# jchibane/Box2Mask

Measured on AMD Instinct MI355X. Metric: ScanNet scenes/sec (fwd+bwd, ~150k voxels @2cm), higher is better.
Workload: dtype f32; 1 GPU; ScanNet 2cm voxels, batch_size=8 per GPU, sparse-conv fwd/bwd + losses + Adam (BASELINE configs[1]); global_batch=8, ranks_seen=1, voxels_per_gpu_batch=1202778, parallelism=dp1, distinct_batches=4, setup_steps=2, prefetch=next batch: coordinate + kernel maps on a second stream during the step, steps_executed=51, full=False

## Files before the change

box2mask_amd/_lib.py:

```python
from __future__ import annotations

import ctypes as C
import os

import torch

_HERE = os.path.dirname(os.path.abspath(__file__))
LIB_PATH = os.environ.get('B2M_LIB_PATH', os.path.join(_HERE, 'libb2m_hip.so'))

P = C.c_void_p
I32 = C.c_int32
I64 = C.c_int64
F32 = C.c_float
F64 = C.c_double

PROTOTYPES = {
    'b2m_coords_build': [P, I64, P, P, I64, P, P],
    'b2m_morton_keys': [P, I64, P, P],
    'b2m_hilbert_keys': [P, I64, I32, P, P],
    'b2m_coords_stride': [P, I64, I32, P, P, P, P, P, I64, P, C.POINTER(I64), P],
    'b2m_kernel_map': [P, I64, I32, I32, P, P, I64, P, I32, I32, I32, P, I64, P],
    'b2m_occupancy': [P, I64, I32, I32, I32, I32, P, I64, P],
    'b2m_kernel_map_rulebook': [P, I64, I32, I32, P, P, I64, P, I32, I32, I32, P, P, P, P],
    'b2m_stride_tables': [P, P, I64, I64, P, I64, P, I64, P],
# ... 21 lines not shown
    'b2m_weight_pack_run': [P, I32, I64, P],
    'b2m_weight_pack_h_run': [P, I32, I64, P],
    'b2m_conv_wgrad': [P, I64, I32, I64, P, I64, I32, P, P, P, I64, I32, P, I64, I64, P, P],
    'b2m_conv_wgrad_tr': [P, I64, I32, I64, P, I64, I32, P, P, P, I64, I32, P, I64, I64, P, P],
    'b2m_bn_stats': [P, I64, I64, I32, P, P, P],
    'b2m_bn_tilestats': [P, I64, I32, P, P, P],
    'b2m_bn_tilestats_finalize': [P, I64, I64, I32, P, P, P, P, F32, F32, P, P, P, P, P, P, P],
    'b2m_bn_finalize': [P, F64, P, I32, P, P, F32, F32, P, P, P, P, P, P, P],
    'b2m_bn_apply': [P, I64, I64, I32, P, P, P, I64, I32, P, I64, P],
    'b2m_bn_bwd_reduce': [P, I64, P, I64, P, I64, I64, I32, P, P, I32, P, P, P, P, P, P, P],
    'b2m_bn_stats_finalize': [P, I64, I64, I32, P, P, P, P, F32, F32, P, P, P, P, P, P, P],
    'b2m_bn_bwd_apply': [P, I64, P, I64, P, I64, I64, I32, P, P, P, P, F64, P, I32, P, P, P, I64, P, I64, P],
    'b2m_bn_apply2': [P, I64, P, I64, I64, I32, P, P, P, P, I32, P, I64, P],
    'b2m_bn_bwd_reduce2': [P, I64, P, I64, P, I64, P, I64, I64, I32, P, P, P, P, I32, P, P, P],
    'b2m_bn_bwd_apply2': [P, I64, P, I64, P, I64, P, I64, I64, I32, P, P, P, P, P, P, P, F64, P, I32, P, I64, P, I64, P, P, P, P, P, P],
    'b2m_bn_small_fwd': [P, I64, I64, I32, P, P, F32, F32, P, P, P, P, P, P, P, I64, I32, P, I64, P],
    'b2m_bn_small_fwd_stats': [P, I64, I64, I32, P, P],
    'b2m_bn_small_fwd_apply': [P, P, I64, I64, I32, P, P, F32, F32, P, P, P, P, P, P, P, I64, I32, P, I64, P],
    'b2m_bn_small_bwd_phase': [I32, P, I64, P, I64, P, I64, I64, I32, P, P, P, I32, P, P, P, P, P, I64, P, I64, P, P, P],
    'b2m_bn_small_bwd': [P, I64, P, I64, P, I64, I64, I32, P, P, P, I32, P, P, P, P, P, I64, P, I64, P],
    'b2m_relu_fwd': [P, I64, P, P],
    'b2m_relu_bwd': [P, P, I64, P, P],
    'b2m_add': [P, P, I64, P, P],
    'b2m_segment_pool_fwd': [P, I64, I64, I32, P, I64, I32, P, P, P, P, P],
    'b2m_segment_mean_sorted': [P, I64, I64, I32, P, P, I64, P, P, P],
    'b2m_segment_pool_bwd': [P, I64, I32, P, I64, I32, P, P, P, I64, P],
    'b2m_nmc': [P, I32, F32, I32, P, P, P, P, P, P],
    'b2m_nmc_batch': [P, P, I32, I32, F32, P, P, P, P, P, P],
    'b2m_mask_project': [P, I32, P, I32, P, P, I64, F32, P, I64, P],
    'b2m_mask_nms': [P, I32, I64, F32, P, P, P, P],
    'b2m_label_hist': [P, I64, P, I32, P, I64, I32, P, P],
    'b2m_mask_gather': [P, I64, P, I32, P, I64, P, P],
    'b2m_mask_project_batch': [P, I32, I64, I64, F32, P],
    'b2m_mask_nms_batch': [P, I32, I32, F32, P],
    'b2m_label_hist_batch': [P, I32, I64, I32, P],
    'b2m_mask_gather_batch': [P, I32, I64, I64, P],
    'b2m_mask_gather_batch_t': [P, I32, I64, I64, I64, P, P],
    'b2m_mask_nms_sweep': [P, I32, I64, P, I32, P, P, P],
    'b2m_mask_nms_sweep_batch': [P, I32, I32, P, I32, P, I64, P],
    'b2m_mask_hist_index': [P, I64, I32, I64, P, P, I64, I32, P, P, P],
    'b2m_mask_hist_index_batch': [P, I32, I64, I64, P],
    'b2m_mask_hist': [P, I64, I32, P, I64, I32, P, P],
    'b2m_mask_pack': [P, I32, I64, P, I64, P],
    'b2m_set_ious': [P, P, I64, P, P],
    'b2m_mask_hulls': [P, I64, I32, P, I64, P, P, P, I32, P, P, P, P, P, P, P],
    'b2m_obb_corners': [P, P, P, I32, P, P],
    'b2m_hull_box_iou': [P, P, P, P, I32, P, P, I32, P, P],
    'b2m_aabb_iou': [P, P, I32, P, P, P, I32, P, P],
    'b2m_dbscan': [P, I64, I32, F64, I32, P, P, P, P],
    'b2m_paint_proposals': [P, I64, I32, P, I64, I32, F64, I32, P, P, P, P, P],
    'b2m_joint_hist': [P, P, I64, I32, I32, P, P],
    'b2m_vox_shift': [P, I64, P, P, P],
    'b2m_unique_insert_async': [P, I64, P, I64, P, P, P, P],
    'b2m_vox_keys': [P, I64, P, F64, P, P, P],
    'b2m_sort_u64': [P, I64, P],
    'b2m_unique_rank': [P, I64, P, P, I64, P, I64, P, P],
    'b2m_vox_decode': [P, I64, I32, P, P],
    'b2m_vox_nearest': [P, I64, P, F64, P, P, I64, I64, P, P, P],
    'b2m_vox_gather': [P, I64, P, P, P, P, P, P],
    'b2m_seg_centroid': [P, P, I64, I64, F64, P, P, P, P, P],
    'b2m_box_membership': [P, I64, P, P, P, I32, P, P, P, P],
    'b2m_seg_box_vote': [P, I64, P, P, I64, I64, P, P, P, P, I32, P, P, P, P, P],
    'b2m_obb_membership': [P, I64, P, P, P, I32, P, P, P],
    'b2m_seg_rank': [P, I64, P, P, I64, P, P],
    'b2m_seg_mode': [P, P, I64, I64, I32, P, P, P],
    'b2m_aug_stats': [P, I64, P, P, P],
    'b2m_aug_affine': [P, P, I64, P, P, P, P, I32, P],
    'b2m_aug_axpy': [P, P, F64, I64, P],
    'b2m_aug_blur': [P, P, I32, I32, I32, P],
    'b2m_aug_displace': [P, I64, P, I32, I32, I32, P, P, P, F64, P],
    'b2m_aug_vertex_normals': [P, I64, P, I64, P, P, P, P],
    'b2m_aug_colour': [P, I64, P, I32, F64, P, P, P],
    'b2m_inst_boxes': [P, P, P, I64, I64, P, P, P, P, P, P, P, P, P, P],
    'b2m_nn_build': [P, I64, P, P],
    'b2m_nn_query': [P, I64, P, P, I64, P, P, P],
    'b2m_ap_rows': [P, I32, I32, P],
    'b2m_ap_match': [P, I32, I64, P, P, P, I32, P, I64, P, P, P, I64, P, P, P, I32, P],
    'b2m_ap_curve': [P, I64, P, P, I32, P, I64, I64, P, P, P, P],
}
PLAIN = {'b2m_last_error': (C.c_char_p, []), 'b2m_version': (C.c_int, []), 'b2m_device_ok': (C.c_int, []),
         'b2m_reload_env': (C.c_int, []),
         'b2m_weight_pack_size': (C.c_int64, [I32, I32, I32]),
         'b2m_conv_wgrad_workspace': (C.c_int64, [I32, I32, I32]),
         'b2m_weight_pack_h_size': (C.c_int64, [I32, I32, I32, I32]),
         'b2m_unique_insert': (C.c_int64, [P, I64, P, I64, P, P, P, P]),
         'b2m_weight_pack_plan_size': (C.c_int32, []),
         'b2m_weight_pack_h_plan_size': (C.c_int32, []),
         'b2m_weight_pack_h_plan': (C.c_int64, [I32, P, P, P, P, P, P, P, P, P, P, P]),
         'b2m_rulebook_cnt_size': (C.c_int64, [I32, I64]),
         'b2m_radix_argsort_scratch': (C.c_int64, [I64]),
         'b2m_dbscan_workspace': (C.c_int64, [I64]),
         'b2m_nn_workspace': (C.c_int64, [I64]),
         'b2m_xchg_size': (C.c_int64, []), 'b2m_xchg_max_doubles': (C.c_int32, []), 'b2m_xchg_max_ranks': (C.c_int32, []),
         'b2m_xchg_alloc': (C.c_int, [C.POINTER(C.c_void_p), P]), 'b2m_xchg_open': (C.c_int, [P, C.POINTER(C.c_void_p)]),
         'b2m_xchg_close': (C.c_int, [P]), 'b2m_xchg_free': (C.c_int, [P]),
         'b2m_xchg_is_finegrained': (C.c_int32, [P]),
         'b2m_weight_pack_plan': (C.c_int64, [I32, P, P, P, P, P, P, P, P, P, P, P])}

_lib = None


class B2MError(RuntimeError):
    pass


def load():
    global _lib
    if _lib is not None:
        return _lib
    if not os.path.exists(LIB_PATH):
        raise ImportError(
            'box2mask_amd: the HIP extension %s is missing. Build it with '
            '`python -m box2mask_amd.build` (hipcc --offload-arch=gfx950); there is no CPU fallback.' % LIB_PATH)
    lib = C.CDLL(LIB_PATH)
    for name, args in PROTOTYPES.items():
        fn = getattr(lib, name)
        fn.argtypes = args
        fn.restype = C.c_int
    for name, (res, args) in PLAIN.items():
        fn = getattr(lib, name)
        fn.argtypes = args
        fn.restype = res
    _lib = lib
    return lib


def ptr(t):
    if t is None:
        return None
    return t.data_ptr()


_raw_stream = getattr(torch._C, '_cuda_getCurrentRawStream', None)
_raw_device = getattr(torch._C, '_cuda_getDevice', None)


def stream():
    if _raw_stream is not None and _raw_device is not None:
        return _raw_stream(_raw_device())
    return torch.cuda.current_stream().cuda_stream


_hook = None


def set_hook(fn):
    global _hook
    _hook = fn


def call(name, *args, meta=None):
    lib = _lib if _lib is not None else load()
    done = _hook(name, args, meta) if _hook is not None else None
    rc = getattr(lib, name)(*args, stream())
    if done is not None:
        done()
    if rc != 0:
        raise B2MError('%s failed (%d): %s' % (name, rc, lib.b2m_last_error().decode()))


def call_ret(name, *args):
    lib = load()
    done = _hook(name, args, None) if _hook is not None else None
    rc = getattr(lib, name)(*args, stream())
    if done is not None:
        done()
# ... 18 lines not shown
```

box2mask_amd/csrc/conv.hip:

```cpp
#include "b2m_common.h"
#include <stdlib.h>
#include <type_traits>

struct ConvArgs {
    const float* x1; int64_t ldx1; int c1;
    const float* x2; int64_t ldx2; int c2;
    const float* wp; int K;
    const float* bias;
    const int32_t* rb_in; const uint8_t* rb_out; const int32_t* rb_cnt;
    int64_t n_out, ntiles;
    float* y; int64_t ldy; int cout; int accumulate; int nstrips; int vec_store;
    int nslice;
    int chain;
    int fast32;
    const float* zeros;
    int ncs;
    int wg_combine;
    int64_t nwg;
    int64_t xcd_per;
    const int32_t* xcd_start;
    int64_t wg_per_tile;
    const int32_t* tile_order;
    double* stats;
    const float* ep_scale; const float* ep_shift; const float* ep_res; int64_t ld_res; int ep_relu;
// ... 509 lines not shown
        bool more = true;
        while (more) {
#pragma unroll
            for (int u = 0; u < 3; ++u) {
                if (k0 < 0) { more = false; break; }
                const int n = count_of(k0);
                const int G = (n + 15) >> 4;
                const int k2c = valid(k2, valid(k1, k0)), k3c = valid(k3, k2c);
                load_ops(k2c, idx, av[(u + 2) % 3], w[(u + 2) % 3]);
                load_idx(k3c, idx);
                f32x4 acc[NG][TW];
#pragma unroll
                for (int g = 0; g < NG; ++g) {
                    if (g < G) {
#pragma unroll
                        for (int t = 0; t < TW; ++t) {
                            f32x4 c = {0.f, 0.f, 0.f, 0.f};
                            c = __builtin_amdgcn_mfma_f32_16x16x4f32(av[u][g][0], w[u][t], c, 0, 0, 0);
                            acc[g][t] = __builtin_amdgcn_mfma_f32_16x16x4f32(av[u][g][1], w[u][2 + t], c, 0, 0, 0);
                        }
                    }
                }
#pragma unroll
                for (int g = 0; g < NG; ++g) {
                    if (g < G) {
                        int ad[4];
                        float old[4][TW];
#pragma unroll
                        for (int r = 0; r < 4; ++r) {
                            ad[r] = (16 * g + 4 * q + r < n) ? (int)((out[u][g] >> (8 * r)) & 255) : B2M_TILE;
#pragma unroll
                            for (int t = 0; t < TW; ++t) old[r][t] = Cs[cs_index<TW>(ad[r], 16 * t + i)];
                        }
#pragma unroll
                        for (int r = 0; r < 4; ++r)
#pragma unroll
                            for (int t = 0; t < TW; ++t) Cs[cs_index<TW>(ad[r], 16 * t + i)] = old[r][t] + acc[g][t][r];
                    }
                }
                load_out(k3c, out[u]);
                k0 = k1; k1 = k2; k2 = k3;
                k3 = k2 < 0 ? -1 : next_active(k2);
            }
        }
        __builtin_amdgcn_fence(__ATOMIC_SEQ_CST, "wavefront");
    }
    if (a.stats && lane < a.cout) {
        const int64_t rem = a.n_out - row0;
        const int rows = rem < B2M_TILE ? (int)rem : B2M_TILE;
        double s1[4] = {0., 0., 0., 0.}, s2[4] = {0., 0., 0., 0.};
        int r = 0;
        for (; r + 3 < rows; r += 4) {
#pragma unroll
            for (int u = 0; u < 4; ++u) {
                const double v = (double)Cs[cs_index<TW>(r + u, lane)];
                s1[u] += v; s2[u] = fma(v, v, s2[u]);
            }
        }
        for (; r < rows; ++r) {
            const double v = (double)Cs[cs_index<TW>(r, lane)];
            s1[0] += v; s2[0] = fma(v, v, s2[0]);
        }
        double* o = a.stats + tile * 2 * a.cout + lane;
        o[0] = (s1[0] + s1[1]) + (s1[2] + s1[3]); o[a.cout] = (s2[0] + s2[1]) + (s2[2] + s2[3]);
    }
    for (int e = lane; e < B2M_TILE * (SW / 4); e += 64) {
        const int row = e / (SW / 4), c4 = (e % (SW / 4)) * 4;
        const int64_t grow = row0 + row;
        if (grow >= a.n_out) continue;
        f32x4 v = *(const f32x4*)&Cs[cs_index<TW>(row, c4)];
        float* dst = a.y + grow * a.ldy + c4;
        if (a.vec_store && c4 + 3 < a.cout) {
            if constexpr (EP) v = conv_epilogue(a, v, grow, c4);
            *(f32x4*)dst = v;
        } else {
#pragma unroll
            for (int u = 0; u < 4; ++u) if (c4 + u < a.cout) dst[u] = v[u];
        }
    }
}

#include "conv_fwd_flow.h"
#include "conv_1x1.h"

static inline int conv_kc(int cin) { return cin >= 16 ? 16 : 8; }
static inline int conv_tw(int cout, int K) { return (cout % 48 == 0 && K > 1 && b2m_env_int("B2M_CONV_TW3", 1)) ? 3 : 2; }

extern "C" int64_t b2m_weight_pack_size(int32_t K, int32_t cin, int32_t cout) {
    const int KC = conv_kc(cin);
    const int TW = conv_tw(cout, K);
    const int64_t nchunk = (cin + KC - 1) / KC, nstrip = (cout + 16 * TW - 1) / (16 * TW);
    return (int64_t)K * nstrip * nchunk * (64 * TW * (KC / 4));
}

__global__ void weight_pack_kernel(const float* __restrict__ w, int64_t ldw, int K, int rows, int cols, int transpose,
                                   int mirror, int sb, int CI, int CO, int KC, int TW, float* __restrict__ wp) {
    const int KS = KC / 4, LW = 64 * TW * KS, SW = 16 * TW;
    const int nchunk = (CI + KC - 1) / KC, nstrip = (CO + SW - 1) / SW;
    const int64_t total = (int64_t)K * nstrip * nchunk * LW;
    for (int64_t e = (int64_t)blockIdx.x * blockDim.x + threadIdx.x; e < total; e += (int64_t)gridDim.x * blockDim.x) {
        int lane, f;
        pack_unpos((int)(e % LW), TW * KS, lane, f);
        const int64_t blk = e / LW;
        const int chunk = (int)(blk % nchunk); const int64_t b2 = blk / nchunk;
        const int strip = (int)(b2 % nstrip); const int k = (int)(b2 / nstrip);
        const int s = f / TW, t = f % TW, q = lane >> 4, i = lane & 15;
        const int ci = chunk * KC + KS * q + s, co = strip * SW + 16 * t + i;
        float v = 0.f;
        if (ci < CI && co < CO) {
            if (!transpose) v = w[((int64_t)k * rows + ci) * ldw + co];
            else v = w[((int64_t)(mirror ? K - 1 - k : k) * rows + sb + co) * ldw + ci];
        }
        wp[e] = v;
    }
}
extern "C" int b2m_weight_pack(const float* w, int64_t ldw, int32_t K, int32_t cin, int32_t cout, int32_t transpose,
                               int32_t mirror, int32_t slice_begin, int32_t slice_count, float* wp, void* stream) {
    hipStream_t st = (hipStream_t)stream;
    B2M_CHECK_ARG(w && wp && K >= 1 && cin > 0 && cout > 0 && ldw >= cout, "bad arguments");
    int CI, CO;
    if (!transpose) { CI = cin; CO = cout; }
    else {
        B2M_CHECK_ARG(slice_begin >= 0 && slice_count > 0 && slice_begin + slice_count <= cin, "bad channel slice");
        CI = cout; CO = slice_count;
    }
    const int64_t total = b2m_weight_pack_size(K, CI, CO);
    int64_t grid = (total + 255) / 256;
    if (grid > 65536) grid = 65536;
    weight_pack_kernel<<<(unsigned)grid, 256, 0, st>>>(w, ldw, K, cin, cout, transpose, mirror, slice_begin, CI, CO,
                                                       conv_kc(CI), conv_tw(CO, K), wp);
    B2M_LAUNCH_CHECK();
    return B2M_OK;
}

struct PackDesc {
    const float* w; float* wp;
    int64_t ldw, first_block, total;
    int32_t K, rows, cols, transpose, mirror, sb, CI, CO, KC, TW;
};
extern "C" int32_t b2m_weight_pack_plan_size(void) { return (int32_t)sizeof(PackDesc); }
extern "C" int64_t b2m_weight_pack_plan(int32_t n, const int64_t* w, const int64_t* wp, const int64_t* ldw,
                                        const int32_t* K, const int32_t* cin, const int32_t* cout,
                                        const int32_t* transpose, const int32_t* mirror, const int32_t* slice_begin,
                                        const int32_t* slice_count, void* plan_host) {
    B2M_CHECK_ARG(n >= 0 && (n == 0 || (w && wp && ldw && K && cin && cout && transpose && mirror && slice_begin &&
                                        slice_count && plan_host)), "bad arguments");
    PackDesc* d = (PackDesc*)plan_host;
    int64_t blocks = 0;
    for (int i = 0; i < n; ++i) {
        B2M_CHECK_ARG(w[i] && wp[i] && K[i] >= 1 && cin[i] > 0 && cout[i] > 0 && ldw[i] >= cout[i], "bad layer");
        PackDesc e;
        e.w = (const float*)(uintptr_t)w[i]; e.wp = (float*)(uintptr_t)wp[i]; e.ldw = ldw[i];
        e.K = K[i]; e.rows = cin[i]; e.cols = cout[i]; e.transpose = transpose[i]; e.mirror = mirror[i]; e.sb = slice_begin[i];
        if (!transpose[i]) { e.CI = cin[i]; e.CO = cout[i]; }
        else {
            B2M_CHECK_ARG(slice_begin[i] >= 0 && slice_count[i] > 0 && slice_begin[i] + slice_count[i] <= cin[i], "bad channel slice");
            e.CI = cout[i]; e.CO = slice_count[i];
        }
        e.KC = conv_kc(e.CI); e.TW = conv_tw(e.CO, e.K);
        e.total = b2m_weight_pack_size(e.K, e.CI, e.CO);
        e.first_block = blocks;
        blocks += e.total / (64 * e.TW * (e.KC / 4));
        d[i] = e;
    }
    return blocks;
}
// ... 99 lines not shown
    return rows < (1 << 24) && ld < (1 << 22) && rows * ld * esz < (1ll << 32);
}
static inline bool addr32(int64_t rows, int64_t ld1, int64_t ld2, int esz) { return addr32(rows, ld1, esz) && addr32(rows, ld2, esz); }
static inline ConvArgs conv_args(const float* x1, int64_t ldx1, int c1, const float* x2, int64_t ldx2, int c2, const float* wp, int K,
                                 const int32_t* rb_in, const uint8_t* rb_out, const int32_t* rb_cnt, int64_t n_out, float* y, int64_t ldy,
                                 int cout, int TW) {
    ConvArgs a{};
    a.x1 = x1; a.ldx1 = ldx1; a.c1 = c1; a.x2 = x2; a.ldx2 = ldx2; a.c2 = c2;
    a.wp = wp; a.K = K;
    a.rb_in = rb_in; a.rb_out = rb_out; a.rb_cnt = rb_cnt;
    a.n_out = n_out; a.ntiles = cdiv64(n_out, B2M_TILE);
    a.y = y; a.ldy = ldy; a.cout = cout;
    a.nstrips = (cout + 16 * TW - 1) / (16 * TW);
    return a;
}
static inline unsigned conv_xcd_plan(ConvArgs& a, int64_t items_per_tile, int wpb, bool balanced) {
    const int64_t xcd_tiles = b2m_env_int("B2M_XCD", 1) ? (1 << 30) : 0;
    const XcdOrder o = xcd_order(a.nwg, xcd_tiles * items_per_tile / wpb);
    a.xcd_per = o.chunk;
    if (!(balanced && a.ntiles >= B2M_BALANCE_MIN_TILES && xcd_tiles > 0 && b2m_env_int("B2M_XCD_BALANCE", 1))) return o.grid;
    a.xcd_start = a.rb_cnt + (int64_t)a.K * a.ntiles;
    a.tile_order = b2m_env_int("B2M_XCD_ORDER", 1) ? a.xcd_start + 16 + a.ntiles : nullptr;
    a.wg_per_tile = items_per_tile / wpb;
    return (unsigned)(8 * B2M_XCD_CAP(a.ntiles) * a.wg_per_tile);
}

struct ConvEpilogue { const float* scale; const float* shift; const float* res; int64_t ld_res; int relu; };
static int conv_fwd_impl(const float* x1, int64_t ldx1, int32_t c1, const float* x2, int64_t ldx2, int32_t c2,
                         int64_t n_in, const float* wp, int32_t K, const float* bias, const int32_t* rb_in,
                         const uint8_t* rb_out, const int32_t* rb_cnt, int64_t n_out, float* y, int64_t ldy,
                         int32_t cout, int32_t accumulate, double* tile_stats, int32_t* wrote_stats, void* stream,
                         const ConvEpilogue* ep = nullptr, int32_t* fused = nullptr) {
    hipStream_t st = (hipStream_t)stream;
    if (wrote_stats) *wrote_stats = 0;
    if (fused) *fused = 0;
    B2M_CHECK_ARG(c1 > 0 && c2 >= 0 && cout > 0 && K >= 1 && K <= 128 && n_in >= 0 && n_out >= 0, "bad sizes (K<=128)");
    B2M_CHECK_ARG(ldy >= cout && ldx1 >= c1 && (c2 == 0 || ldx2 >= c2), "leading dimension too small");
    const int cin = c1 + c2;
    const int KC = conv_kc(cin);
    const int KS = KC / 4;
    B2M_CHECK_ARG(c2 == 0 || c1 % KC == 0, "with two sources c1 must be a multiple of 16");
    if (n_out == 0) return B2M_OK;
    B2M_CHECK_ARG(n_in >= 1, "n_in (rows of x1/x2) must be >= 1 where there are output rows");
    B2M_CHECK_ARG(x1 && wp && y, "bad pointers");
    B2M_CHECK_ARG((rb_in == nullptr) == (rb_out == nullptr) && (rb_in == nullptr) == (rb_cnt == nullptr),
                  "rulebook pointers must be all set or all NULL");
    B2M_CHECK_ARG(rb_in != nullptr || K == 1, "identity rulebook needs K == 1");
    B2M_CHECK_ARG(c2 == 0 || x2 != nullptr, "x2 is NULL");
    B2M_CHECK_ARG(((uintptr_t)wp % 16) == 0, "packed weights must be 16-byte aligned");
    const bool fast = c1 % KC == 0 && c2 % KC == 0 && ldx1 % KS == 0 && (c2 == 0 || ldx2 % KS == 0) &&
                      ((uintptr_t)x1 % (4 * KS)) == 0 && ((uintptr_t)x2 % (4 * KS)) == 0;
    const int TW = conv_tw(cout, K);
    ConvArgs a = conv_args(x1, ldx1, c1, x2, ldx2, c2, wp, K, rb_in, rb_out, rb_cnt, n_out, y, ldy, cout, TW);
    a.bias = bias; a.accumulate = accumulate;
    a.vec_store = (ldy % 4 == 0 && ((uintptr_t)y % 16) == 0) ? 1 : 0;
    const bool ep_ok = ep && ep->scale && ep->shift && a.vec_store && cout % 4 == 0 && !accumulate && !bias &&
                       ((uintptr_t)ep->scale % 16) == 0 && ((uintptr_t)ep->shift % 16) == 0 &&
                       (!ep->res || (ep->ld_res % 4 == 0 && ep->ld_res >= cout && ((uintptr_t)ep->res % 16) == 0));
    auto use_epilogue = [&]() {
        a.ep_scale = ep->scale; a.ep_shift = ep->shift; a.ep_res = ep->res; a.ld_res = ep->ld_res; a.ep_relu = ep->relu;
        if (fused) *fused = 1;
    };
    const int64_t items0 = a.ntiles * a.nstrips;
    int nslice = 1;
    const int64_t target = b2m_env_int("B2M_DETERMINISTIC", 0) ? 0 : b2m_env_int("B2M_CONV_TARGET", cin <= 32 ? 4096 : 6144);
    if (items0 < target && K > 1) {
        nslice = (int)cdiv64(target, items0);
        if (nslice > 16) nslice = 16;
        if (nslice > K) nslice = K;
        if (K >= 4 && nslice > 1) {
            nslice = (nslice + 3) / 4 * 4;
            if (nslice > K) nslice = K / 4 * 4;
            if (nslice > 16) nslice = 16;
            const int cap = b2m_env_int("B2M_CONV_MAXSLICE", a.ntiles >= 8 ? 4 : 16);
            if (nslice > cap) nslice = cap;
        }
    }
    int ncs = 1;
    const int nchunk_h = (cin + KC - 1) / KC;
    while (nslice > 1 && ncs < 4 && items0 * nslice * ncs < b2m_env_int("B2M_CONV_CHUNK_ITEMS", 2048) && nchunk_h / (ncs * 2) >= 2 &&
           b2m_env_int("B2M_CONV_CHUNKSPLIT", 1)) ncs *= 2;
    nslice *= ncs;
    a.fast32 = (addr32(n_in, ldx1, ldx2, 4) && b2m_env_int("B2M_CONV_FAST32", 1)) ? 1 : 0;
    bool split2 = false;
    if (nslice == 1 && K >= 8 && rb_in != nullptr && fast && KC == 16 && a.fast32 && (cin / 16) % 2 == 0 && cin >= 32 &&
        b2m_env_int("B2M_CONV_PIPE", 2) && b2m_env_int("B2M_CONV_HANDLOADS", 1) && !b2m_env_int("B2M_PIPE_DBG", 0) &&
        !b2m_env_int("B2M_DETERMINISTIC", 0) && items0 >= target && items0 < b2m_env_int("B2M_CONV_SPLIT2", 0)) {
        nslice = 2;
        split2 = true;
    }
    a.ncs = ncs;
    a.nslice = nslice;
    a.wg_combine = ((nslice > 1 && nslice % 4 == 0 && b2m_env_int("B2M_CONV_WGCOMBINE", 1)) || split2) ? 1 : 0;
    static const float* zeros_addr = nullptr;
    if (!zeros_addr) B2M_HIP(hipGetSymbolAddress((void**)&zeros_addr, HIP_SYMBOL(g_zeros)));
    a.zeros = zeros_addr;
    if (nslice > 1 && !accumulate && !(a.wg_combine && (nslice == 4 || split2)))
        B2M_HIP(hipMemset2DAsync(y, (size_t)ldy * sizeof(float), 0, (size_t)cout * sizeof(float), (size_t)n_out, st));
    const int64_t items = items0 * nslice;
    a.nwg = cdiv64(items, 4);
    const unsigned grid = conv_xcd_plan(a, (int64_t)a.nstrips * nslice, 4, false);
    const bool ident = rb_in == nullptr;
    if (ident && fast && KC == 16 && a.fast32 && n_in >= n_out && b2m_env_int("B2M_CONV_1X1", 1)) {
        int spw = a.nstrips % 3 == 0 ? 3 : a.nstrips % 2 == 0 ? 2 : 1;
        if (a.ntiles * (a.nstrips / spw) < 2048) spw = 1;
        const int64_t g1 = a.ntiles * (a.nstrips / spw);
        B2M_CHECK_ARG(g1 < (1ll << 31), "too many workgroups");
        if (ep_ok) use_epilogue();
        if (spw == 3) conv_1x1_kernel<3><<<(unsigned)g1, 64, 0, st>>>(a);
        else if (spw == 2) conv_1x1_kernel<2><<<(unsigned)g1, 64, 0, st>>>(a);
        else conv_1x1_kernel<1><<<(unsigned)g1, 64, 0, st>>>(a);
        B2M_LAUNCH_CHECK();
        return B2M_OK;
    }
    {
        const int nc = cin / 16;
        const int depth = b2m_env_int("B2M_CONV_PIPE", 2) ? 2 : 0;
        const bool split_ok = nslice == 1 || (a.wg_combine && b2m_env_int("B2M_CONV_FLOW_SPLIT", 1));
        if (depth >= 2 && !ident && fast && KC == 16 && split_ok && a.fast32 && nc % ncs == 0 && (nc / ncs) % depth == 0 &&
            nc / ncs >= depth) {
            const int wpb = nslice == 1 ? 1 : split2 ? 2 : 4;
            B2M_CHECK_ARG(items0 < (1ll << 31), "too many (tile, strip) items");
            a.chain = (wpb == 1 && b2m_env_int("B2M_CONV_CHAIN", 1)) ? 1 : 0;
            if (tile_stats && (nslice == 1 || ((nslice == 4 || split2) && !accumulate))) {
                a.stats = tile_stats;
                if (wrote_stats) *wrote_stats = 1;
            }
            if (ep_ok && (nslice == 1 || nslice == 4 || split2)) use_epilogue();
            a.nwg = cdiv64(items, wpb);
            const unsigned fgrid = conv_xcd_plan(a, (int64_t)a.nstrips * nslice, wpb, (a.nstrips * nslice) % wpb == 0);
            const int dbg = b2m_env_int("B2M_PIPE_DBG", 0);
            const int hl = b2m_env_int("B2M_CONV_HANDLOADS", 1);
            if (hl && depth == 2 && dbg == 32 && wpb == 1 && TW == 3) {
                conv_fwd_flow_kernel<2, 3, 32, 1, 1><<<fgrid, 64, 0, st>>>(a);
                B2M_LAUNCH_CHECK();
                return B2M_OK;
            }
            if (hl && depth == 2 && dbg == 8 && wpb == 1 && TW == 3) {
                conv_fwd_flow_kernel<2, 3, 8, 1, 1><<<fgrid, 64, 0, st>>>(a);
                B2M_LAUNCH_CHECK();
                return B2M_OK;
            }
            if (hl && depth == 2 && !dbg) {
                if (wpb == 2) {
                    if (TW == 3) conv_fwd_flow_kernel<2, 3, 0, 2, 1><<<fgrid, 128, 0, st>>>(a);
                    else conv_fwd_flow_kernel<2, 2, 0, 2, 1><<<fgrid, 128, 0, st>>>(a);
                } else if (wpb == 4) {
                    if (TW == 3) conv_fwd_flow_kernel<2, 3, 0, 4, 1><<<fgrid, 256, 0, st>>>(a);
                    else conv_fwd_flow_kernel<2, 2, 0, 4, 1><<<fgrid, 256, 0, st>>>(a);
                } else {
                    if (TW == 3) conv_fwd_flow_kernel<2, 3, 0, 1, 1><<<fgrid, 64, 0, st>>>(a);
                    else conv_fwd_flow_kernel<2, 2, 0, 1, 1><<<fgrid, 64, 0, st>>>(a);
                }
                B2M_LAUNCH_CHECK();
                return B2M_OK;
            }
            if (wpb == 4) {
                if (TW == 3) conv_fwd_flow_kernel<2, 3, 0, 4><<<fgrid, 256, 0, st>>>(a);
                else conv_fwd_flow_kernel<2, 2, 0, 4><<<fgrid, 256, 0, st>>>(a);
            } else if (dbg && TW == 3) {
                switch (dbg) {
                    case 1: conv_fwd_flow_kernel<2, 3, 1><<<fgrid, 64, 0, st>>>(a); break;
                    case 2: conv_fwd_flow_kernel<2, 3, 2><<<fgrid, 64, 0, st>>>(a); break;
                    case 4: conv_fwd_flow_kernel<2, 3, 4><<<fgrid, 64, 0, st>>>(a); break;
                    case 8: conv_fwd_flow_kernel<2, 3, 8><<<fgrid, 64, 0, st>>>(a); break;
                    default: conv_fwd_flow_kernel<2, 3, 6><<<fgrid, 64, 0, st>>>(a); break;
// ... 1259 lines not shown
```

box2mask_amd/functional.py:

```python
from __future__ import annotations

import ctypes
import itertools
import os
import weakref

import torch
import torch.distributed as dist

from . import _lib
from .grad_arena import grad_slot
from .sparse import Rulebook

_call = _lib.call
_ptr = _lib.ptr


def deterministic() -> bool:
    return os.environ.get('B2M_DETERMINISTIC', '0') == '1'


_wgrad_ws = {}


# ... 104 lines not shown
        for k in keys:
            if k[1]:
                back.append(k)
                continue
            size += self.entries[k][2].numel() * 4
            (early if size <= self.EARLY_BYTES else late).append(k)
        self.split = (self._plan_of(early), self._plan_of(late), self._plan_of(back))
        self.group = {k: g for g, ks in enumerate((early, late, back)) for k in ks}

    def begin_pass(self, inference=False):
        if self.env_epoch != _lib.env_epoch[0]:
            self.__init__()
        if inference and not self.dirty and self.plan is not None and getattr(self, '_epoch', None) == training_epoch():
            return
        self._epoch = training_epoch()
        self.pass_id += 1
        if not self.entries:
            return
        if self.dirty or any(e[0]() is None or e[0]().data_ptr() != e[4] for e in self.entries.values()):
            self._build_plan()
        if self.plan is None:
            return
        plan, n, blocks, keys = self.plan
        self.pending = {}
        dev = plan.device
        if not inference and pack_on_side_stream() and wgrad_on_side_stream() and torch.is_grad_enabled():
            main, side = torch.cuda.current_stream(dev), _side_stream(dev)
            early, late, back = self.split
            if early is not None:
                _call('b2m_weight_pack_run', early[0].data_ptr(), early[1], early[2])
            side.wait_stream(main)
            with torch.cuda.stream(side):
                for g, pl in ((1, late), (2, back)):
                    if pl is not None:
                        _call('b2m_weight_pack_run', pl[0].data_ptr(), pl[1], pl[2])
                        ev = torch.cuda.Event()
                        ev.record(side)
                        self.pending[g] = ev
        else:
            _call('b2m_weight_pack_run', plan.data_ptr(), n, blocks)
        for k in keys:
            e = self.entries[k]
            e[3], e[5] = e[0]()._version, self.pass_id

    def join(self):
        for g in list(self.pending):
            torch.cuda.current_stream().wait_event(self.pending.pop(g))


def pack_on_side_stream() -> bool:
    return os.environ.get('B2M_PACK_STREAM', '1') == '1'


packed_weights = _PackedWeights()


class _ZeroSlab:
    CHUNK = 4 << 20

    def __init__(self):
        self.chunk = {}

    def new_pass(self):
        self.chunk.clear()

    def take(self, n, c, device):
        need = (n * c + 63) // 64 * 64
        if need > self.CHUNK // 4:
            return None
        e = self.chunk.get(device)
        if e is None or e[1] + need > e[0].numel():
            e = [torch.zeros(self.CHUNK, dtype=torch.float32, device=device), 0]
            self.chunk[device] = e
        t = e[0][e[1]:e[1] + n * c].view(n, c)
        e[1] += need
        t._b2m_slab = True
        return t


zero_slab = _ZeroSlab()
TINY_MAP_ROWS = 8 * 64


def conv_zero_slab() -> bool:
    return os.environ.get('B2M_CONV_ZERO_SLAB', '1') == '1'


def conv_raw(x1, x2, wp, K: int, bias, rb: Rulebook | None, n_out: int, cout: int, out=None, accumulate=False,
             tile_stats: list | None = None, logical_cin: int | None = None):
    c1 = x1.shape[1]
    c2 = x2.shape[1] if x2 is not None else 0
    if out is None and rb is not None and K > 1 and 0 < n_out < TINY_MAP_ROWS and not deterministic() and conv_zero_slab():
        out = zero_slab.take(n_out, cout, x1.device)
        accumulate = out is not None
    if out is None:
        out = torch.empty((n_out, cout), dtype=torch.float32, device=x1.device)
    meta = None if logical_cin is None else {'cin': logical_cin}
    if rb is None:
        assert K == 1
        rbi = rbo = rbc = None
    else:
        assert rb.K == K and rb.n_out == n_out
        rbi, rbo, rbc = rb.rb_in.data_ptr(), rb.rb_out.data_ptr(), rb.rb_cnt.data_ptr()
    if rb is not None and rb.scatter is not None and n_out > 0 and x1.shape[0] > 0:
        sc = rb.scatter
        assert sc.K == K and sc.n_out == x1.shape[0]
        ran = ctypes.c_int32(0)
        m_up = {'ran': ran}
        if logical_cin is not None:
            m_up['cin'] = logical_cin
        _call('b2m_conv_up', x1.data_ptr(), x1.stride(0), c1, _ptr(x2), x2.stride(0) if x2 is not None else 0, c2, x1.shape[0],
              wp.data_ptr(), K, _ptr(bias), sc.rb_in.data_ptr(), sc.rb_out.data_ptr(), sc.rb_cnt.data_ptr(), out.data_ptr(),
              out.stride(0), cout, n_out, 1 if accumulate else 0, None, None, None, 0, 0, ctypes.byref(ran), meta=m_up)
        if ran.value:
            return out
    if tile_stats is not None and rb is not None and n_out > 0:
        ntiles = (n_out + 63) // 64
        ts = torch.empty((ntiles, 2, cout), dtype=torch.float64, device=x1.device)
        wrote = ctypes.c_int32(0)
        _call('b2m_conv_fwd_stats', x1.data_ptr(), x1.stride(0), c1, _ptr(x2), x2.stride(0) if x2 is not None else 0, c2,
              x1.shape[0], wp.data_ptr(), K, _ptr(bias), rbi, rbo, rbc, n_out, out.data_ptr(), out.stride(0), cout,
              1 if accumulate else 0, ts.data_ptr(), ctypes.byref(wrote), meta=meta)
        if wrote.value:
            tile_stats.append((ts, ntiles))
        return out
    _call('b2m_conv_fwd', x1.data_ptr(), x1.stride(0), c1, _ptr(x2), x2.stride(0) if x2 is not None else 0, c2,
          x1.shape[0], wp.data_ptr(), K, _ptr(bias), rbi, rbo, rbc, n_out, out.data_ptr(), out.stride(0), cout,
          1 if accumulate else 0, meta=meta)
    return out


_half_images = {}
_half_epoch = [0]


def note_training_pass():
    _half_epoch[0] += 1


def training_epoch() -> int:
    return _half_epoch[0]


invalidate_half_images = note_training_pass


def _after_optimizer_step(optimizer, args, kwargs):
    note_training_pass()


try:
    from torch.optim.optimizer import register_optimizer_step_post_hook as _reg_post_hook
    _reg_post_hook(_after_optimizer_step)
except ImportError:
    pass



def weight_pack_h(weight, c1: int, c2: int):
    w3 = weight.detach()
    w3 = w3 if w3.dim() == 3 else w3.unsqueeze(0)
    assert w3.dtype == torch.float32 and w3.is_contiguous()
    K, cin, cout = w3.shape
    assert cin == c1 + c2
    e = _half_images.get(id(weight))
    if (e is not None and e[0]() is weight and e[1] == (c1, c2) and e[3] == weight._version and e[4] == weight.data_ptr()
            and e[5] == (_half_epoch[0], _lib.env_epoch[0])):
        return e[2]
    n = _lib.load().b2m_weight_pack_h_size(K, c1, c2, cout)
    image = torch.empty(n, dtype=torch.float16, device=w3.device)
    _call('b2m_weight_pack_h', w3.data_ptr(), cout, K, c1, c2, cout, image.data_ptr())
    if e is None:
        for k in [k for k, v in _half_images.items() if v[0]() is None]:
            del _half_images[k]
    _half_images[id(weight)] = [weakref.ref(weight), (c1, c2), image, weight._version, weight.data_ptr(), (_half_epoch[0], _lib.env_epoch[0])]
# ... 767 lines not shown
```

include/b2m.h:

```cpp
#ifndef B2M_H
#define B2M_H
#include <stdint.h>
#ifdef __cplusplus
extern "C" {
#endif

#define B2M_TILE 64
#define B2M_OK 0
#define B2M_ERR_ARG (-1)
#define B2M_ERR_HIP (-2)
#define B2M_ERR_UNSUPPORTED (-3)

const char* b2m_last_error(void);
int b2m_version(void);
int b2m_device_ok(void);
int b2m_reload_env(void);


int b2m_coords_build(const int32_t* coords, int64_t n, uint64_t* keys, int32_t* vals, int64_t cap,
                     int32_t* dup_count, void* stream);

int b2m_morton_keys(const int32_t* coords, int64_t n, int64_t* keys, void* stream);
int b2m_hilbert_keys(const int32_t* coords, int64_t n, int32_t bits, int64_t* keys, void* stream);

int64_t b2m_radix_argsort_scratch(int64_t n);
int b2m_radix_argsort(const uint64_t* keys, int64_t n, uint64_t bit_mask, int64_t* perm, int64_t* inv_perm, void* scratch,
                      void* stream);

int b2m_coords_stride(const int32_t* coords, int64_t n, int32_t ts,
                      int32_t* coords_out, int32_t* parent, int32_t* koff,
                      uint64_t* keys, int32_t* vals, int64_t cap,
                      int32_t* scratch, int64_t* n_out_host, void* stream);

int b2m_kernel_map(const int32_t* coords, int64_t n, int32_t ksize, int32_t ts,
                   const uint64_t* keys, const int32_t* vals, int64_t cap,
                   const uint64_t* occ, int32_t dim_x, int32_t dim_y, int32_t dim_z,
                   int32_t* nbr, int64_t ld, void* stream);

int b2m_kernel_map_rulebook(const int32_t* coords, int64_t n, int32_t ksize, int32_t ts,
                            const uint64_t* keys, const int32_t* vals, int64_t cap,
                            const uint64_t* occ, int32_t dim_x, int32_t dim_y, int32_t dim_z,
                            int32_t* rb_in, uint8_t* rb_out, int32_t* rb_cnt, void* stream);

int b2m_occupancy(const int32_t* coords, int64_t n, int32_t batches, int32_t dim_x, int32_t dim_y, int32_t dim_z,
                  uint64_t* bits, int64_t words, void* stream);

int b2m_stride_tables(const int32_t* parent, const int32_t* koff, int64_t n_fine, int64_t n_coarse,
                      int32_t* child, int64_t ld_c, int32_t* up, int64_t ld_f, void* stream);

int64_t b2m_rulebook_cnt_size(int32_t K, int64_t n_out);
int b2m_rulebook_balance(int32_t* rb_cnt, int32_t K, int64_t n_out, void* stream);
int b2m_rulebook(const int32_t* nbr, int64_t ld, int32_t K, int64_t n_out,
                 int32_t* rb_in, uint8_t* rb_out, int32_t* rb_cnt, int32_t* pair_total, void* stream);

int b2m_detection_loss(const float* off, int64_t ld_off, const float* bnd, int64_t ld_bnd, const float* sc, int64_t ld_sc,
                       const float* sem, int64_t ld_sem, int32_t n_class, const float* gt_off, const float* gt_bnd,
                       const float* loc, const uint8_t* fg, const int64_t* gt_sem, int64_t S, double n_fg,
                       const double* n_valid, float w_off, float w_bnd, float w_sc, float w_sem, float min_bb_size,
                       float* d_off, float* d_bnd, float* d_sc, float* d_sem, int64_t* argmax, double* sums,
                       float* result, void* stream);


int64_t b2m_weight_pack_size(int32_t K, int32_t cin, int32_t cout);
int b2m_weight_pack(const float* w, int64_t ldw, int32_t K, int32_t cin, int32_t cout, int32_t transpose,
                    int32_t mirror, int32_t slice_begin, int32_t slice_count, float* wp, void* stream);

int32_t b2m_weight_pack_plan_size(void);
int64_t b2m_weight_pack_plan(int32_t n, const int64_t* w, const int64_t* wp, const int64_t* ldw, const int32_t* K,
                             const int32_t* cin, const int32_t* cout, const int32_t* transpose,
                             const int32_t* mirror, const int32_t* slice_begin, const int32_t* slice_count,
                             void* plan_host);
int b2m_weight_pack_run(const void* plan_dev, int32_t n, int64_t total_blocks, void* stream);

int b2m_conv_fwd(const float* x1, int64_t ldx1, int32_t c1, const float* x2, int64_t ldx2, int32_t c2,
                 int64_t n_in, const float* wp, int32_t K, const float* bias,
                 const int32_t* rb_in, const uint8_t* rb_out, const int32_t* rb_cnt,
                 int64_t n_out, float* y, int64_t ldy, int32_t cout, int32_t accumulate, void* stream);

int b2m_conv_fwd_stats(const float* x1, int64_t ldx1, int32_t c1, const float* x2, int64_t ldx2, int32_t c2,
                       int64_t n_in, const float* wp, int32_t K, const float* bias,
                       const int32_t* rb_in, const uint8_t* rb_out, const int32_t* rb_cnt,
                       int64_t n_out, float* y, int64_t ldy, int32_t cout, int32_t accumulate,
                       double* tile_stats, int32_t* wrote_stats, void* stream);

int b2m_conv_fwd_affine(const float* x1, int64_t ldx1, int32_t c1, const float* x2, int64_t ldx2, int32_t c2,
                        int64_t n_in, const float* wp, int32_t K,
                        const int32_t* rb_in, const uint8_t* rb_out, const int32_t* rb_cnt,
                        int64_t n_out, float* y, int64_t ldy, int32_t cout,
                        const float* scale, const float* shift, const float* res, int64_t ld_res, int32_t relu,
                        int32_t* fused, void* stream);

int64_t b2m_weight_pack_h_size(int32_t K, int32_t c1, int32_t c2, int32_t cout);
int b2m_weight_pack_h(const float* w, int64_t ldw, int32_t K, int32_t c1, int32_t c2, int32_t cout, void* wp, void* stream);
int b2m_conv_fwd_h(const void* x1, int64_t ldx1, int32_t c1, const void* x2, int64_t ldx2, int32_t c2, int64_t n_in,
                   const void* wp, int32_t K, const int32_t* rb_in, const uint8_t* rb_out, const int32_t* rb_cnt,
                   int64_t n_out, void* y, int64_t ldy, int32_t cout, const float* scale, const float* shift,
                   const void* res, int64_t ld_res, int32_t relu, void* stream);
int b2m_conv_fwd_h_stats(const void* x1, int64_t ldx1, int32_t c1, const void* x2, int64_t ldx2, int32_t c2, int64_t n_in,
                         const void* wp, int32_t K, const int32_t* rb_in, const uint8_t* rb_out, const int32_t* rb_cnt,
                         int64_t n_out, void* y, int64_t ldy, int32_t cout, double* tile_stats, void* stream);

int b2m_conv_up(const float* x1, int64_t ldx1, int32_t c1, const float* x2, int64_t ldx2, int32_t c2, int64_t n_coarse,
                const float* wp, int32_t K, const float* bias, const int32_t* rb_in, const uint8_t* rb_out,
                const int32_t* rb_cnt, float* y, int64_t ldy, int32_t cout, int64_t n_fine, int32_t accumulate,
                const float* scale, const float* shift, const float* res, int64_t ld_res, int32_t relu,
                int32_t* ran, void* stream);

int64_t b2m_conv_wgrad_workspace(int32_t K, int32_t cin, int32_t cout);
int b2m_conv_wgrad(const float* x, int64_t ldx, int32_t cin, int64_t n_in, const float* dy, int64_t lddy, int32_t cout,
                   const int32_t* rb_in, const uint8_t* rb_out, const int32_t* rb_cnt,
                   int64_t n_out, int32_t K, float* dw, int64_t lddw, int64_t dw_kstride, float* workspace, void* stream);
int b2m_conv_wgrad_tr(const float* x, int64_t ldx, int32_t cin, int64_t n_in, const float* dy, int64_t lddy, int32_t cout,
                   const int32_t* rb_in, const uint8_t* rb_out, const int32_t* rb_cnt,
                   int64_t n_out, int32_t K, float* dw, int64_t lddw, int64_t dw_kstride, float* workspace, void* stream);

int b2m_conv_wgrad_h(const void* x, int64_t ldx, int32_t cin, int64_t n_in, const void* dy, int64_t lddy, int32_t cout,
                     const int32_t* rb_in, const uint8_t* rb_out, const int32_t* rb_cnt, int64_t n_out, int32_t K,
                     float* dw, int64_t lddw, int64_t dw_kstride, int32_t tr, float out_scale, void* stream);
int b2m_weight_pack_h_t(const float* w, int32_t K, int32_t cin, int32_t cout, int32_t mirror, int32_t s0, int32_t sc, void* wp,
                        void* stream);
int32_t b2m_weight_pack_h_plan_size(void);
int64_t b2m_weight_pack_h_plan(int32_t n, const int64_t* w, const int64_t* wp, const int32_t* K, const int32_t* cin, const int32_t* cout,
                               const int32_t* c1, const int32_t* transposed, const int32_t* mirror, const int32_t* s0, const int32_t* sc,
                               void* plan_host);
int b2m_weight_pack_h_run(const void* plan_dev, int32_t n, int64_t total_blocks, void* stream);
int b2m_bn_stats_finalize_h(const void* x, int64_t ldx, int64_t n, int32_t c, double* partial, const float* gamma, const float* beta,
                            float eps, float momentum, float* running_mean, float* running_var, float* mean, float* invstd,
                            float* scale, float* shift, void* stream);
int b2m_bn_stats_h(const void* x, int64_t ldx, int64_t n, int32_t c, double* partial, double* stats, void* stream);
int b2m_bn_apply_h(const void* x, int64_t ldx, int64_t n, int32_t c, const float* scale, const float* shift,
                   const void* residual, int64_t ldr, int32_t relu, void* y, int64_t ldy, void* stream);
int b2m_bn_bwd_reduce_h(const void* dy, int64_t lddy, const void* y, int64_t ldy, const void* x, int64_t ldx, int64_t n,
                        int32_t c, const float* mean, const float* invstd, int32_t relu, const float* mask_scale,
                        const float* mask_shift, double* partial, double* sums,
                        float* dbeta_f32, float* dgamma_f32, float param_grad_scale, void* stream);
int b2m_bn_bwd_apply_h(const void* dy, int64_t lddy, const void* y, int64_t ldy, const void* x, int64_t ldx, int64_t n,
                       int32_t c, const float* mean, const float* invstd, const float* gamma, const double* sums,
                       double count, const double* count_dev, int32_t relu, const float* mask_scale, const float* mask_shift,
                       void* dx, int64_t lddx, void* dres, int64_t lddres, void* stream);

int64_t b2m_xchg_size(void);
int32_t b2m_xchg_max_doubles(void);
int32_t b2m_xchg_max_ranks(void);
int b2m_xchg_alloc(void** buf, void* handle64);
int b2m_xchg_open(const void* handle64, void** ptr);
int b2m_xchg_close(void* ptr);
int b2m_xchg_free(void* buf);
int32_t b2m_xchg_is_finegrained(const void* buf);
int b2m_xchg_allreduce(const double* vals, int32_t n, const void* const* peers_dev, int32_t rank, int32_t world,
                       uint64_t epoch, double* out, int32_t* err, void* stream);

int b2m_clock_probe(unsigned long long* out4, int32_t iters, void* stream);


int b2m_bn_stats(const float* x, int64_t ldx, int64_t n, int32_t c, double* partial, double* stats, void* stream);

int b2m_bn_stats_finalize(const float* x, int64_t ldx, int64_t n, int32_t c, double* partial, double* stats,
                          const float* gamma, const float* beta, float eps, float momentum,
                          float* running_mean, float* running_var, float* mean, float* invstd,
                          float* scale, float* shift, void* stream);

int b2m_bn_tilestats(const double* tile_stats, int64_t ntiles, int32_t c, double* partial, double* stats, void* stream);
int b2m_bn_tilestats_finalize(const double* tile_stats, int64_t ntiles, int64_t n, int32_t c, double* partial,
                              double* stats, const float* gamma, const float* beta, float eps, float momentum,
                              float* running_mean, float* running_var, float* mean, float* invstd, float* scale,
                              float* shift, void* stream);
// ... 164 lines not shown
```

Baseline: 118.2 scenes/s.

## Add dedicated small-output sparse conv kernel splitting work over offsets and channels

Adds a specialized forward conv kernel for outputs of up to 1024 rows (coarse U-Net levels). Each block handles one kernel offset, one output strip and one channel range. It stages that weight slice in LDS, runs MFMA over rulebook pairs, and atomically accumulates into a zeroed output. This is meant to expose more parallelism than the tile-based path on tiny maps, where few tiles leave most CUs idle. The Python side widens the zero-slab threshold so these outputs arrive pre-zeroed. The cost is heavy float atomics, non-deterministic sums, and a per-call path counter.

```diff
diff --git a/box2mask_amd/_lib.py b/box2mask_amd/_lib.py
--- a/box2mask_amd/_lib.py
+++ b/box2mask_amd/_lib.py
@@ -127,6 +127,7 @@
          'b2m_reload_env': (C.c_int, []),
          'b2m_weight_pack_size': (C.c_int64, [I32, I32, I32]),
          'b2m_conv_wgrad_workspace': (C.c_int64, [I32, I32, I32]),
+         'b2m_conv_path_count': (C.c_int64, [I32, I32]),
          'b2m_weight_pack_h_size': (C.c_int64, [I32, I32, I32, I32]),
          'b2m_unique_insert': (C.c_int64, [P, I64, P, I64, P, P, P, P]),
          'b2m_weight_pack_plan_size': (C.c_int32, []),
diff --git a/box2mask_amd/csrc/conv.hip b/box2mask_amd/csrc/conv.hip
--- a/box2mask_amd/csrc/conv.hip
+++ b/box2mask_amd/csrc/conv.hip
@@ -615,6 +615,7 @@
 
 #include "conv_fwd_flow.h"
 #include "conv_1x1.h"
+#include "conv_small.h"
 
 static inline int conv_kc(int cin) { return cin >= 16 ? 16 : 8; }
 static inline int conv_tw(int cout, int K) { return (cout % 48 == 0 && K > 1 && b2m_env_int("B2M_CONV_TW3", 1)) ? 3 : 2; }
@@ -880,6 +881,12 @@
            b2m_env_int("B2M_CONV_CHUNKSPLIT", 1)) ncs *= 2;
     nslice *= ncs;
     a.fast32 = (addr32(n_in, ldx1, ldx2, 4) && b2m_env_int("B2M_CONV_FAST32", 1)) ? 1 : 0;
+    if (rb_in != nullptr && K > 1 && n_out <= conv_small_rows() && fast && KC == 16 && a.fast32 && a.vec_store && cout % 16 == 0 &&
+        !ep && !b2m_env_int("B2M_DETERMINISTIC", 0)) {
+        a.nslice = 1; a.ncs = 1;
+        return conv_small_launch(a, TW, st);
+    }
+    g_conv_path[B2M_CONV_PATH_OTHER].fetch_add(1);
     bool split2 = false;
     if (nslice == 1 && K >= 8 && rb_in != nullptr && fast && KC == 16 && a.fast32 && (cin / 16) % 2 == 0 && cin >= 32 &&
         b2m_env_int("B2M_CONV_PIPE", 2) && b2m_env_int("B2M_CONV_HANDLOADS", 1) && !b2m_env_int("B2M_PIPE_DBG", 0) &&
diff --git a/box2mask_amd/csrc/conv_small.h b/box2mask_amd/csrc/conv_small.h
--- /dev/null
+++ b/box2mask_amd/csrc/conv_small.h
@@ -0,0 +1,160 @@
+#pragma once
+#include "conv_small_index.h"
+
+struct CsUnit { int tl, g, n, row; uint32_t out; };
+__device__ __forceinline__ CsUnit cs_fetch_unit(const ConvArgs& a, const CsPlan& p, const CsBlock& b, int j, int g0, int g1, int g2, int g3,
+                                                int n0, int n1, int n2, int n3, int lane) {
+    CsUnit u = {0, 0, 0, 0, 0u};
+    int tl = 0, g = 0;
+    if (!cs_unit(j, g0, g1, g2, g3, tl, g)) return u;
+    u.tl = tl; u.g = g;
+    u.n = tl == 0 ? n0 : tl == 1 ? n1 : tl == 2 ? n2 : n3;
+    const int64_t tile = b.t_lo + tl;
+    const int pa = cs_pair_a(g, lane);
+    int row = 0;
+    if (pa < u.n) row = a.rb_in[cs_slot(p, b.k, tile, pa)];
+    u.row = row < 0 ? 0 : row;
+    u.out = *(const uint32_t*)(a.rb_out + cs_slot(p, b.k, tile, cs_pair_d(g, lane, 0)));
+    return u;
+}
+
+template <int TW, int NB, int WAVES>
+__global__ __launch_bounds__(64 * WAVES) void conv_small_kernel(ConvArgs a, CsPlan p) {
+    extern __shared__ __attribute__((aligned(16))) float cs_w[];
+    constexpr int LW = 64 * TW * 4;
+    const int tid = threadIdx.x, lane = tid & 63, wave = tid >> 6;
+    const CsBlock b = cs_block(p, blockIdx.x);
+    const int nch1 = a.c1 / 16;
+
+    const float* wsrc = a.wp + cs_weight_offset(p, b);
+    const int nfl = cs_weight_floats(p, b);
+    constexpr int NR = CS_CPW * LW / (64 * WAVES * 4);
+    f32x4 wv[NR];
+#pragma unroll
+    for (int r = 0; r < NR; ++r) {
+        const int e = cs_copy_offset(r, tid, WAVES);
+        wv[r] = e < nfl ? *(const f32x4*)(wsrc + e) : f32x4{0.f, 0.f, 0.f, 0.f};
+    }
+
+    int n_t[CS_TPW];
+#pragma unroll
+    for (int tl = 0; tl < CS_TPW; ++tl) {
+        const int64_t tile = b.t_lo + tl;
+        int n = tile < b.t_hi ? a.rb_cnt[cs_cnt_index(p, b.k, tile)] : 0;
+        n_t[tl] = n < 0 ? 0 : n > CS_TILE ? CS_TILE : n;
+    }
+    const int g0 = cs_groups(n_t[0]), g1 = cs_groups(n_t[1]), g2 = cs_groups(n_t[2]), g3 = cs_groups(n_t[3]);
+    const int total = g0 + g1 + g2 + g3;
+
+    if (a.bias && b.k == 0 && b.cr == 0) {
+        const int64_t r_lo = b.t_lo * CS_TILE;
+        const int64_t r_hi = b.t_hi * CS_TILE < a.n_out ? b.t_hi * CS_TILE : a.n_out;
+        const int nrow = (int)(r_hi - r_lo);
+        for (int e = tid; e < nrow * 16 * TW; e += 64 * WAVES) {
+            const int col = b.strip * 16 * TW + e % (16 * TW);
+            if (col < a.cout) atomicAdd(a.y + (r_lo + e / (16 * TW)) * a.ldy + col, a.bias[col]);
+        }
+    }
+    if (total == 0) return;
+
+    CsUnit nx = cs_fetch_unit(a, p, b, wave, g0, g1, g2, g3, n_t[0], n_t[1], n_t[2], n_t[3], lane);
+
+#pragma unroll
+    for (int r = 0; r < NR; ++r) {
+        const int e = cs_copy_offset(r, tid, WAVES);
+        if (e < nfl) *(f32x4*)(cs_w + e) = wv[r];
+    }
+    __syncthreads();
+
+    for (int j = wave; j < total; j += WAVES) {
+        const int g = nx.g, n = nx.n, row = nx.row;
+        const int64_t tile = b.t_lo + nx.tl;
+        const uint32_t out4 = nx.out;
+
+        f32x4 acc[2][TW];
+#pragma unroll
+        for (int h = 0; h < 2; ++h)
+#pragma unroll
+            for (int t = 0; t < TW; ++t) acc[h][t] = f32x4{0.f, 0.f, 0.f, 0.f};
+
+        for (int c0 = b.c_lo; c0 < b.c_hi; c0 += NB) {
+            f32x4 av[NB];
+#pragma unroll
+            for (int jj = 0; jj < NB; ++jj) {
+                const int c = c0 + jj < b.c_hi ? c0 + jj : b.c_hi - 1;
+                const float* src = cs_second_source(c, nch1) ? a.x2 + cs_a_offset(row, a.ldx2, c, nch1, lane)
+                                                              : a.x1 + cs_a_offset(row, a.ldx1, c, nch1, lane);
+                av[jj] = *(const f32x4*)src;
+            }
+            if (c0 == b.c_lo) nx = cs_fetch_unit(a, p, b, j + WAVES, g0, g1, g2, g3, n_t[0], n_t[1], n_t[2], n_t[3], lane);
+#pragma unroll
+            for (int jj = 0; jj < NB; ++jj) {
+                if (c0 + jj < b.c_hi) {
+                    const int cl = c0 + jj - b.c_lo;
+                    float w[TW * 4];
+#pragma unroll
+                    for (int u = 0; u < TW; ++u) {
+                        const f32x4 w4 = *(const f32x4*)(cs_w + cs_lds_frag(TW, cl, u, lane));
+                        w[4 * u] = w4[0]; w[4 * u + 1] = w4[1]; w[4 * u + 2] = w4[2]; w[4 * u + 3] = w4[3];
+                    }
+#pragma unroll
+                    for (int s = 0; s < 4; ++s)
+#pragma unroll
+                        for (int t = 0; t < TW; ++t)
+                            acc[s & 1][t] = __builtin_amdgcn_mfma_f32_16x16x4f32(av[jj][s], w[TW * s + t], acc[s & 1][t], 0, 0, 0);
+                }
+            }
+        }
+
+#pragma unroll
+        for (int t = 0; t < TW; ++t) {
+            const int col = cs_col(TW, b.strip, t, lane);
+            if (col < a.cout) {
+#pragma unroll
+                for (int r = 0; r < 4; ++r) {
+                    const int orow = (int)((out4 >> (8 * r)) & 255);
+                    if (cs_pair_d(g, lane, r) < n && orow < CS_TILE && tile * CS_TILE + orow < a.n_out)
+                        atomicAdd(a.y + cs_y_offset(tile, orow, a.ldy, col), acc[0][t][r] + acc[1][t][r]);
+                }
+            }
+        }
+    }
+}
+
+#include <atomic>
+static std::atomic<long long> g_conv_path[B2M_CONV_PATHS];
+extern "C" int64_t b2m_conv_path_count(int32_t which, int32_t reset) {
+    if (which < 0 || which >= B2M_CONV_PATHS) return -1;
+    return reset ? g_conv_path[which].exchange(0) : g_conv_path[which].load();
+}
+
+static inline int conv_small_rows() { return b2m_env_int("B2M_CONV_SMALL_ROWS", 1024); }
+
+template <int TW, int WAVES>
+static void conv_small_launch_nb(const ConvArgs& a, const CsPlan& p, hipStream_t st) {
+    const size_t lds = (size_t)cs_lds_floats(TW) * sizeof(float);
+    if (p.nchunk <= 4) conv_small_kernel<TW, 4, WAVES><<<(unsigned)p.grid, 64 * WAVES, lds, st>>>(a, p);
+    else conv_small_kernel<TW, 16, WAVES><<<(unsigned)p.grid, 64 * WAVES, lds, st>>>(a, p);
+}
+template <int TW>
+static void conv_small_launch_waves(const ConvArgs& a, const CsPlan& p, hipStream_t st) {
+    if (p.waves == 16) conv_small_launch_nb<TW, 16>(a, p, st);
+    else if (p.waves == 8) conv_small_launch_nb<TW, 8>(a, p, st);
+    else conv_small_launch_nb<TW, 4>(a, p, st);
+}
+
+static int conv_small_launch(const ConvArgs& a, int TW, hipStream_t st) {
+    const int64_t ntiles = cdiv64(a.n_out, CS_TILE);
+    int tpw = b2m_env_int("B2M_CONV_SMALL_TPW", 0), waves = b2m_env_int("B2M_CONV_SMALL_WAVES", 0);
+    if (tpw <= 0) tpw = (ntiles > 4 && a.K > 8) ? 2 : 1;
+    if (waves <= 0) waves = ntiles == 1 ? 16 : 4;
+    const CsPlan p = cs_plan(a.K, a.c1 + a.c2, a.cout, a.n_out, TW, tpw, waves);
+    B2M_CHECK_ARG(p.grid > 0 && p.grid < (1ll << 31), "bad grid");
+    if (!a.accumulate)
+        B2M_HIP(hipMemset2DAsync(a.y, (size_t)a.ldy * sizeof(float), 0, (size_t)a.cout * sizeof(float), (size_t)a.n_out, st));
+    if (TW == 3) conv_small_launch_waves<3>(a, p, st);
+    else conv_small_launch_waves<2>(a, p, st);
+    B2M_LAUNCH_CHECK();
+    g_conv_path[B2M_CONV_PATH_SMALL].fetch_add(1);
+    return B2M_OK;
+}
diff --git a/box2mask_amd/csrc/conv_small_index.h b/box2mask_amd/csrc/conv_small_index.h
--- /dev/null
+++ b/box2mask_amd/csrc/conv_small_index.h
@@ -0,0 +1,81 @@
+#pragma once
+#include <stdint.h>
+
+#if defined(__HIPCC__) || defined(__CUDACC__)
+#define CS_HD __host__ __device__ __forceinline__
+#else
+#define CS_HD static inline
+#endif
+
+#define CS_TILE 64
+#define CS_TPW 4
+#define CS_CPW 16
+#define CS_MAX_WAVES 16
+
+struct CsPlan {
+    int K, TW, nstrips, nchunk, ncr, nparts, tpw, waves;
+    int64_t ntiles;
+    int64_t nws;
+    int64_t grid;
+};
+struct CsBlock { int k, strip, cr, part, c_lo, c_hi; int64_t t_lo, t_hi; };
+
+CS_HD int cs_lw(int TW) { return 64 * TW * 4; }
+CS_HD int cs_lds_floats(int TW) { return CS_CPW * cs_lw(TW); }
+
+CS_HD CsPlan cs_plan(int K, int cin, int cout, int64_t n_out, int TW, int tpw, int waves) {
+    CsPlan p;
+    p.K = K; p.TW = TW;
+    p.tpw = tpw < 1 ? 1 : tpw > CS_TPW ? CS_TPW : tpw;
+    p.waves = waves >= 16 ? 16 : waves >= 8 ? 8 : 4;
+    p.nstrips = (cout + 16 * TW - 1) / (16 * TW);
+    p.nchunk = cin / 16;
+    p.ncr = (p.nchunk + CS_CPW - 1) / CS_CPW;
+    p.ntiles = (n_out + CS_TILE - 1) / CS_TILE;
+    p.nparts = (int)((p.ntiles + p.tpw - 1) / p.tpw);
+    p.nws = (int64_t)K * p.nstrips * p.ncr;
+    p.grid = p.nws * p.nparts;
+    return p;
+}
+CS_HD CsBlock cs_block(const CsPlan& p, int64_t id) {
+    CsBlock b;
+    b.part = (int)(id / p.nws);
+    int64_t ws = id % p.nws;
+    b.cr = (int)(ws % p.ncr); ws /= p.ncr;
+    b.strip = (int)(ws % p.nstrips);
+    b.k = (int)(ws / p.nstrips);
+    b.c_lo = b.cr * CS_CPW;
+    b.c_hi = b.c_lo + CS_CPW < p.nchunk ? b.c_lo + CS_CPW : p.nchunk;
+    b.t_lo = (int64_t)b.part * p.tpw;
+    b.t_hi = b.t_lo + p.tpw < p.ntiles ? b.t_lo + p.tpw : p.ntiles;
+    return b;
+}
+CS_HD int64_t cs_weight_offset(const CsPlan& p, const CsBlock& b) {
+    return (((int64_t)b.k * p.nstrips + b.strip) * p.nchunk + b.c_lo) * cs_lw(p.TW);
+}
+CS_HD int cs_weight_floats(const CsPlan& p, const CsBlock& b) { return (b.c_hi - b.c_lo) * cs_lw(p.TW); }
+CS_HD int cs_copy_offset(int r, int tid, int waves) { return (r * 64 * waves + tid) * 4; }
+CS_HD int cs_copy_rounds(int TW, int waves) { return cs_lds_floats(TW) / (64 * waves * 4); }
+CS_HD int cs_lds_frag(int TW, int cl, int u, int lane) { return cl * cs_lw(TW) + u * 256 + lane * 4; }
+
+CS_HD int64_t cs_cnt_index(const CsPlan& p, int k, int64_t tile) { return (int64_t)k * p.ntiles + tile; }
+CS_HD int64_t cs_slot(const CsPlan& p, int k, int64_t tile, int pair) { return ((int64_t)k * p.ntiles + tile) * CS_TILE + pair; }
+CS_HD int cs_groups(int n) { return n <= 0 ? 0 : n >= CS_TILE ? CS_TILE / 16 : (n + 15) >> 4; }
+CS_HD bool cs_unit(int j, int g0, int g1, int g2, int g3, int& tl, int& g) {
+    if (j < g0) { tl = 0; g = j; return true; }
+    j -= g0;
+    if (j < g1) { tl = 1; g = j; return true; }
+    j -= g1;
+    if (j < g2) { tl = 2; g = j; return true; }
+    j -= g2;
+    if (j < g3) { tl = 3; g = j; return true; }
+    return false;
+}
+CS_HD int cs_pair_a(int g, int lane) { return 16 * g + (lane & 15); }
+CS_HD bool cs_second_source(int c, int nch1) { return c >= nch1; }
+CS_HD int64_t cs_a_offset(int64_t row, int64_t ld, int c, int nch1, int lane) {
+    return row * ld + (int64_t)(c >= nch1 ? c - nch1 : c) * 16 + 4 * (lane >> 4);
+}
+CS_HD int cs_pair_d(int g, int lane, int r) { return 16 * g + 4 * (lane >> 4) + r; }
+CS_HD int cs_col(int TW, int strip, int t, int lane) { return strip * 16 * TW + 16 * t + (lane & 15); }
+CS_HD int64_t cs_y_offset(int64_t tile, int orow, int64_t ldy, int col) { return (tile * CS_TILE + orow) * ldy + col; }
diff --git a/box2mask_amd/functional.py b/box2mask_amd/functional.py
--- a/box2mask_amd/functional.py
+++ b/box2mask_amd/functional.py
@@ -210,6 +210,14 @@
 TINY_MAP_ROWS = 8 * 64
 
 
+def conv_small_rows() -> int:
+    return int(os.environ.get('B2M_CONV_SMALL_ROWS', '1024'))
+
+
+def zeroed_output_rows() -> int:
+    return max(TINY_MAP_ROWS, conv_small_rows() + 1)
+
+
 def conv_zero_slab() -> bool:
     return os.environ.get('B2M_CONV_ZERO_SLAB', '1') == '1'
 
@@ -218,7 +226,7 @@
              tile_stats: list | None = None, logical_cin: int | None = None):
     c1 = x1.shape[1]
     c2 = x2.shape[1] if x2 is not None else 0
-    if out is None and rb is not None and K > 1 and 0 < n_out < TINY_MAP_ROWS and not deterministic() and conv_zero_slab():
+    if out is None and rb is not None and K > 1 and 0 < n_out < zeroed_output_rows() and not deterministic() and conv_zero_slab():
         out = zero_slab.take(n_out, cout, x1.device)
         accumulate = out is not None
     if out is None:
diff --git a/include/b2m.h b/include/b2m.h
--- a/include/b2m.h
+++ b/include/b2m.h
@@ -82,6 +82,11 @@
                        const int32_t* rb_in, const uint8_t* rb_out, const int32_t* rb_cnt,
                        int64_t n_out, float* y, int64_t ldy, int32_t cout, int32_t accumulate,
                        double* tile_stats, int32_t* wrote_stats, void* stream);
+
+#define B2M_CONV_PATH_SMALL 0
+#define B2M_CONV_PATH_OTHER 1
+#define B2M_CONV_PATHS 2
+int64_t b2m_conv_path_count(int32_t which, int32_t reset);
 
 int b2m_conv_fwd_affine(const float* x1, int64_t ldx1, int32_t c1, const float* x2, int64_t ldx2, int32_t c2,
                         int64_t n_in, const float* wp, int32_t K,
```

Result: no change. 118.8 scenes/s (median of 6 runs) (+0.5%).
